# yuki-inaho/APDe-MVS

Measured on AMD Instinct MI355X. Metric: Mpix/s per PatchMatch iteration (ref view, N src) at 1/2/4/8 GPU; depth L1 vs ref, higher is better.
Workload: dtype f32

## Files before the change

### apde-mvs_amd/csrc/apd_kernels.hip

```cpp
#include <hip/hip_runtime.h>

#include <algorithm>
#include <cmath>
#include <cstdio>
#include <cstring>
#include <string>
#include <atomic>
#include <vector>

#include "../../include/apd_hip.h"
#include "apd_device.h"
#include <rocprim/device/device_scan.hpp>

using namespace apd;

#define WAVE 64
#define BLOCK 256
#define APD_PROF_SLOTS 64
#define APD_INSTR 32
#define APD_PROF_SPREAD 64
#define PROF_AT(ev, k) ((ev) + (k) + APD_PROF_SLOTS * (blockIdx.x & (APD_PROF_SPREAD - 1)))
#ifdef APD_PHASE_STAMPS
#define PHASE_STAMP(i)                                                                       \
    do {                                                                                     \
// ... 1876 lines not shown
        if (!live) continue;
        if (nwa) ++*nwa;
        if (inv == 0.0f) continue;
        const float c = ncc_finalize_pre(inv, srp, var, ss, sss, srs);
#pragma unroll
        for (int t = 0; t < 9; ++t) if (t == ns) sc[t] = c;
        ns++;
        strong_weight += 1.0f;
    }
    if (dead) return APD_COST_MAX;
    if (strong_weight <= 1e-6f) return center_cost;
    float mx = -1e10f;
#pragma unroll
    for (int t = 0; t < 9; ++t) if (t < ns && sc[t] > mx) mx = sc[t];
    float e[9];
    float sum = 0.0f;
#pragma unroll
    for (int t = 0; t < 9; ++t) {
        if (t < ns) { e[t] = d_expf(sc[t] - mx); sum += e[t]; }
    }
    float acc = 0.0f;
#pragma unroll
    for (int t = 0; t < 9; ++t) {
        if (t < ns) { float w = e[t] / sum; acc = fmaf(w, sc[t], acc); }
    }
    acc = (acc > APD_COST_MAX) ? APD_COST_MAX : acc;
    return (float)(0.25 * (double)center_cost + 0.75 * (double)acc);
}

#ifndef WV_WAVES
#define WV_WAVES 4
#endif
#ifndef WV_CUR_MATCH
#define WV_CUR_MATCH 1
#endif
#ifndef WV_P2_GEOM_BATCH
#define WV_P2_GEOM_BATCH 0
#endif
#define WV_BLOCK (WV_WAVES * WAVE)
__device__ __forceinline__ size_t cand_at(bool gm, int N, int v, int h, int wc, int wi, int li) {
    return gm ? ((size_t)(li / VM_P) * (size_t)(N * 8) + (size_t)(v * 8 + h)) * VM_P + (size_t)(li % VM_P)
              : ((size_t)v * 8 + h) * (size_t)wc + (size_t)wi;
}
#define GP_NO_FOCAL (-1.0f)
__device__ __forceinline__ float gp_focal(const float (&sc)[8]) {
    uint32_t pm = 0;
    float strong_weight = 0.0f;
#pragma unroll
    for (int k = 0; k < 8; ++k)
        if (sc[k] >= 0.0f) { pm |= 1u << k; strong_weight += 1.0f; }
    if (strong_weight <= 1e-6f) return GP_NO_FOCAL;
    float mx = -1e10f;
#pragma unroll
    for (int k = 0; k < 8; ++k) if (((pm >> k) & 1u) && sc[k] > mx) mx = sc[k];
    float e[8];
    float sum = 0.0f;
#pragma unroll
    for (int k = 0; k < 8; ++k) {
        e[k] = 0.0f;
        if ((pm >> k) & 1u) { e[k] = d_expf(sc[k] - mx); sum += e[k]; }
    }
    float acc = 0.0f;
#pragma unroll
    for (int k = 0; k < 8; ++k)
        if ((pm >> k) & 1u) { const float w = e[k] / sum; acc = fmaf(w, sc[k], acc); }
    acc = (acc > APD_COST_MAX) ? APD_COST_MAX : acc;
    return acc;
}
__device__ __forceinline__ float gp_final(bool dead, float centre_cost, float acc) {
    if (dead) return APD_COST_MAX;
    if (acc < 0.0f) return centre_cost;
    return (float)(0.25 * (double)centre_cost + 0.75 * (double)acc);
}
template <bool F16, bool SA> struct WvOcc {
#ifdef WV_LDS_OCC
    static constexpr int occ = WV_LDS_OCC;
#else
    static constexpr int occ = F16 ? 4 : 3;
#endif
    static constexpr bool pipe = occ < 4 && WV_CENTRE_PIPE;
};
template <bool F16, bool SA>
__global__ __launch_bounds__(WV_BLOCK, (WvOcc<F16, SA>::occ)) void k_sweep_weak_vm(Args a, const int *__restrict__ list, int count,
                                                                int iter, float *cand, int wc, int gm, int centre_in_sweep) {
    const int N = a.N, W = a.W;
    constexpr bool PIPE = WvOcc<F16, SA>::pipe;
    PHASE_BEGIN;
    const bool direct = cand != nullptr;
    WvLdsT<F16, 9, SA> &L = *reinterpret_cast<WvLdsT<F16, 9, SA> *>(apd_dyn_lds);
    wv_init_lut(L);
    float *costL = reinterpret_cast<float *>(&L + 1);
    uint8_t *wts = reinterpret_cast<uint8_t *>(costL + wv_cost_rows(N, direct) * VM_P);
    uint8_t *asl = wts + N * VM_P;
    const int VB = min(WV_P5_CHUNKS, N);
    const int blk = xcd_remap(blockIdx.x, gridDim.x);
    const int first = blk * VM_P;
    const int np = min(VM_P, count - first);
    const int tid = threadIdx.x;
    const int wave = __builtin_amdgcn_readfirstlane(tid >> 6), lane = tid & (WAVE - 1);
    const APD_C Cam &cam0 = a.cams[0];
    const bool geom = a.geom != 0;
    const float gf = a.gf;
    const int p1 = lane;
    const bool pv1 = p1 < np;
    const int c1 = list[first + min(p1, np - 1)];
    const int py1 = c1 / W, px1 = c1 - py1 * W;

    if (pv1) {
        const APD_G short2 *anc = a.anchors + (size_t)a.amap[c1] * 9;
        const int cid = a.sa_any ? a.sa[c1] : 0;
        const bool use_sa = cid != 0;
        if (wave == 0) {
            uint32_t hflag = 0, awin = 0;
            short2 ap[9];
#pragma unroll
            for (int k = 0; k < 9; ++k) ap[k] = anc[k];
            int lab[9], qk[9];
            uint8_t st[9];
            uint32_t sl[9];
#pragma unroll
            for (int k = 0; k < 9; ++k) {
                const bool ok = !(ap[k].x == -1 || ap[k].y == -1);
                qk[k] = ok ? ap[k].x + ap[k].y * W : c1;
                lab[k] = a.sa_any ? (int)a.sa[qk[k]] : cid;
                st[k] = a.weak[qk[k]];
                sl[k] = a.sel[qk[k]];
            }
            for (int v = 0; v < N; ++v) {
                uint32_t b = 0;
#pragma unroll
                for (int k = 1; k < 9; ++k) b |= ((sl[k] >> v) & 1u) << (k - 1);
                asl[v * VM_P + p1] = (uint8_t)b;
            }
            float4 hp[9];
#pragma unroll
            for (int k = 1; k < 9; ++k) hp[k] = a.plane[st[k] == APD_STRONG ? qk[k] : c1];
            const float4 cur = a.plane[c1];
#pragma unroll
            for (int k = 0; k < 9; ++k) {
                const bool ok = !(ap[k].x == -1 || ap[k].y == -1);
                L.anc[k * VM_P + p1] = ok ? ((int)(uint16_t)ap[k].x | ((int)ap[k].y << 16)) : -1;
                if (ok && !(use_sa && lab[k] != cid)) awin |= 1u << k;
                if (k >= 1 && ok && st[k] == APD_STRONG) {
                    hflag |= 1u << (k - 1);
                    L.hyp[(k - 1) * VM_P + p1] = hp[k];
                }
            }
            uint32_t cmatch = 0;
#pragma unroll
            for (int k = 8; k >= 1; --k)
                if (WV_CUR_MATCH && ((hflag >> (k - 1)) & 1u) && __float_as_uint(hp[k].x) == __float_as_uint(cur.x) &&
                    __float_as_uint(hp[k].y) == __float_as_uint(cur.y) && __float_as_uint(hp[k].z) == __float_as_uint(cur.z) &&
                    __float_as_uint(hp[k].w) == __float_as_uint(cur.w))
                    cmatch = (1u << 15) | ((uint32_t)(k - 1) << 12);
            L.flags[p1] = hflag | cmatch | (awin << 16) | (use_sa ? (1u << 29) : 0u);
            LANE_STAT(0, true);
            LANE_STAT(2, cmatch != 0);
#ifdef APD_PHASE_STAMPS
            {
                const float4 ft = a.fit[c1];
                auto same = [](float4 u, float4 w) {
                    return __float_as_uint(u.x) == __float_as_uint(w.x) && __float_as_uint(u.y) == __float_as_uint(w.y) &&
                           __float_as_uint(u.z) == __float_as_uint(w.z) && __float_as_uint(u.w) == __float_as_uint(w.w);
                };
                bool fc = false;
#pragma unroll
                for (int k = 1; k < 9; ++k) fc = fc || (((hflag >> (k - 1)) & 1u) && same(hp[k], ft));
                const bool has_fit = !(ft.x == 0 && ft.y == 0 && ft.z == 0);
                LANE_STAT(4, has_fit && same(ft, cur));
                LANE_STAT(6, has_fit && fc);
            }
#endif
            L.hyp[8 * VM_P + p1] = cur;
            L.pxy[p1] = px1 | (py1 << 16);
            int bx0 = px1, by0 = py1, bx1 = px1, by1 = py1;
#pragma unroll
            for (int k = 0; k < 9; ++k) {
                if (ap[k].x == -1 || ap[k].y == -1) continue;
                bx0 = min(bx0, (int)ap[k].x); bx1 = max(bx1, (int)ap[k].x);
                by0 = min(by0, (int)ap[k].y); by1 = max(by1, (int)ap[k].y);
            }
            L.box[p1] = (uint32_t)bx0 | ((uint32_t)by0 << 16);
            L.box[VM_P + p1] = (uint32_t)bx1 | ((uint32_t)by1 << 16);
        }
        wv_build_windows<F16>(a, L, p1, anc, cid, wave, WV_WAVES);
    }
    __syncthreads();
    PHASE_STAMP(0);

// ... 144 lines not shown
        if (G.valid) {
            wts[v * VM_P + p] = (uint8_t)w;
            if (G.v == 0) {
                const float4 fit = a.fit[c];
                L.st[2 * VM_P + p] = fcm;
                L.st[3 * VM_P + p] = wn;
                L.tsel[p] = tsel;
                uint32_t fl = (L.flags[p] & ~(7u << 25)) | ((uint32_t)mi << 25);
                if (!(fit.x == 0 && fit.y == 0 && fit.z == 0)) fl |= 1u << 31;
                L.flags[p] = fl;
                L.rng_n[p] = (uint16_t)rg.n;
            }
        }
    }
    __syncthreads();

    PHASE_STAMP(22);
    const int cur_row = direct ? 0 : 8 * N;
    const bool cur_shared = WV_CUR_MATCH && pv1 && ((L.flags[p1] >> 15) & 1u);
    for (int v = wave; v < N; v += WV_WAVES) {
        float val = 0.0f;
        const bool want = pv1 && wts[v * VM_P + p1] > 0 && !cur_shared;
        LANE_STAT(24, want);
        if (__ballot(want)) {
            const float4 pl = L.hyp[8 * VM_P + p1];
            const float kept = (iter == 0 && a.wcur && want) ? a.wcur[(size_t)v * a.HW + c1] : __int_as_float(0x7fc00000);
            const bool eval = want && __builtin_isnan(kept);
            float nv = kept;
            if (__ballot(eval)) {
                const float e = ncc_new_vm<F16, SA, true, 9, PIPE>(a, L, p1, px1, py1, v + 1, pl, eval, nullptr, &nwc, &nwa);
                if (eval) nv = e;
            }
            if (want) {
                val = nv;
                if (geom) val = fmaf(gf, geom_cost(a, px1, py1, v + 1, pl), val);
            }
        }
        if (!cur_shared) costL[(cur_row + v) * VM_P + p1] = val;
    }
    __syncthreads();

    if (wave == 0 && pv1) {
        const float wn = L.st[3 * VM_P + p1];
        float cost_now = 0.0f;
        for (int k = 0; k < N; ++k) {
            const int wk = wts[k * VM_P + p1];
            if (wk > 0) cost_now = fmaf((float)wk, costL[(cur_row + k) * VM_P + p1], cost_now);
        }
        cost_now /= wn;
        const float cost_init = cost_now;
        const int mi = (int)((L.flags[p1] >> 25) & 7u);
        const float fcm = L.st[2 * VM_P + p1];
        const float4 cur = L.hyp[8 * VM_P + p1];
        float depth_now = depth_from_plane(cam0, cur, px1, py1);
        float4 pnow = cur;
        bool taken = false;
        if ((L.flags[p1] >> mi) & 1u) {
            const float4 cnd = L.hyp[mi * VM_P + p1];
            const float db = depth_from_plane(cam0, cnd, px1, py1);
            if (db >= a.dmin && db <= a.dmax && fcm < cost_now) {
                depth_now = db; pnow = cnd; cost_now = fcm;
                a.sel[c1] = L.tsel[p1];
                taken = true;
            }
        }
        LANE_STAT(16, taken);
        L.pnow[p1] = pnow;
        L.st[0 * VM_P + p1] = depth_now;
        L.st[1 * VM_P + p1] = cost_now;
        L.st[2 * VM_P + p1] = cost_init;
    }
    __syncthreads();
    PHASE_STAMP(2);
    const bool refine = pv1 && (L.flags[p1] >> 31) != 0u;
    const float4 fit1 = a.fit[c1];
    uint32_t issued_nn = 0, issued_g = 0;

    float *part = reinterpret_cast<float *>(&L.hyp[5 * VM_P]);
    uint8_t *nxt = reinterpret_cast<uint8_t *>(part + 6 * VM_P);
    uint8_t *dead = nxt + 6 * VM_P;
    static_assert(6 * VM_P * (sizeof(float) + 2) <= 3 * VM_P * sizeof(float4), "early-exit state overlays hyp[5..7]");
    for (int i = tid; i < 6 * VM_P; i += WV_BLOCK) { part[i] = 0.0f; nxt[i] = 0; dead[i] = 0; }
    __syncthreads();
    auto fold = [&](int s, int K, int k, int row, int done) {
        for (int p = tid; p < VM_P; p += WV_BLOCK) {
            const int it = s * VM_P + p;
            if (dead[it]) continue;
            int v = nxt[it];
            float P = part[it];
            const int v0 = v;
            for (; v < N && v * K + k < done; ++v) {
                const int wk = wts[v * VM_P + p];
                if (wk > 0) P = fmaf((float)wk, costL[(row + v) * VM_P + p], P);
            }
            if (v == v0) continue;
            nxt[it] = (uint8_t)v;
            part[it] = P;
            if (P / L.st[3 * VM_P + p] >= L.st[1 * VM_P + p]) dead[it] = 1;
        }
    };

    for (int v0 = 0; v0 < N; v0 += WV_WAVES) {
        if (v0 > 0) fold(0, 1, 0, 0, v0);
        const int v = v0 + wave;
        if (v < N) {
            float cv = 0.0f;
            const bool want = refine && wts[v * VM_P + p1] > 0 && !dead[p1];
            LANE_STAT(22, want);
            const float4 fit = fit1;
            const float nv = ncc_new_vm<F16, SA, true, 9, PIPE>(a, L, p1, px1, py1, v + 1, fit, want, nullptr, &nwc, &nwa);
            if (want) {
                cv = nv;
                if (geom) cv = fmaf(gf, geom_cost(a, px1, py1, v + 1, fit), cv);
                ++issued_nn;
                issued_g += geom;
            }
            costL[v * VM_P + p1] = cv;
        }
        __syncthreads();
    }
    PHASE_STAMP(3);

    if (wave == 0 && refine) {
        const float wn = L.st[3 * VM_P + p1];
        float depth_now = L.st[0 * VM_P + p1], cost_now = L.st[1 * VM_P + p1];
        float4 pnow = L.pnow[p1];
        const float4 fit = fit1;
        if (!dead[p1]) {
            float tc = 0.0f;
            for (int kk = 0; kk < N; ++kk) {
                const int wk = wts[kk * VM_P + p1];
                if (wk > 0) tc = fmaf((float)wk, costL[kk * VM_P + p1], tc);
            }
            tc /= wn;
            const float db = depth_from_plane(cam0, fit, px1, py1);
            if (db >= a.dmin && db <= a.dmax && tc < cost_now) { depth_now = db; pnow = fit; cost_now = tc; }
        }
        Rng rg(a.seed_lo, a.seed_hi, (uint32_t)c1, ord_weak(iter));
        rg.n = L.rng_n[p1];
        if (rg.n & 3u) rg.refill();
        const Cands C = refine_candidates(a, px1, py1, rg, pnow, depth_now);
        for (int k = 0; k < 5; ++k) {
            float dk;
            float4 t = candidate(C, k, pnow, depth_now, dk);
            t.w = dist2origin(cam0, px1, py1, dk, t);
            WV_CAND(L)[k * VM_P + p1] = t;
        }
        L.pnow[p1] = pnow;
        L.st[0 * VM_P + p1] = depth_now;
        L.st[1 * VM_P + p1] = cost_now;
    }
    __syncthreads();
    PHASE_STAMP(4);

    {
        auto view_masks = [&](int v, uint64_t (&m)[5]) {
            const bool base = refine && wts[v * VM_P + p1] > 0;
#pragma unroll
            for (int k = 0; k < 5; ++k) m[k] = __ballot(base && !dead[(1 + k) * VM_P + p1]);
        };
        for (int v0 = 0; v0 < N;) {
            int v1 = v0, nch = 0, nne = 0;
            uint64_t ne = 0;
            while (v1 < N && nne < VB && nch < WV_P5_CHUNKS) {
                uint64_t m[5];
                view_masks(v1, m);
                int t = 0;
#pragma unroll
                for (int k = 0; k < 5; ++k) t += __builtin_popcountll(m[k]);
                nch += (t + WAVE - 1) / WAVE;
                if (t > 0) { ne |= 1ull << (v1 - v0); ++nne; }
                ++v1;
            }
            int g = 0;
            for (int v = v0; v < v1; ++v) {
                uint64_t m[5];
                view_masks(v, m);
                int off[6];
                off[0] = 0;
#pragma unroll
                for (int k = 0; k < 5; ++k) off[k + 1] = off[k] + __builtin_popcountll(m[k]);
                const int nv_items = off[5];
                for (int j = 0; j * WAVE < nv_items; ++j, ++g) {
                    if (g % WV_WAVES != wave) continue;
                    const int it = j * WAVE + lane;
                    const bool want = it < nv_items;
                    int k = 0;
#pragma unroll
                    for (int q = 1; q < 5; ++q) k += it >= off[q];
                    uint64_t mk = m[0];
#pragma unroll
                    for (int q = 1; q < 5; ++q) if (k == q) mk = m[q];
                    int pk = 0;
#pragma unroll
                    for (int q = 1; q < 5; ++q) if (k == q) pk = off[q];
                    const int p = want ? nth_set_bit(mk, it - pk) : p1;
                    const int pxy = L.pxy[p];
                    const int px = pxy & 0xFFFF, py = pxy >> 16;
                    const float4 tp = WV_CAND(L)[k * VM_P + p];
                    LANE_STAT(20, want);
                    const float nv = ncc_new_vm<F16, SA, true, 9, PIPE>(a, L, p, px, py, v + 1, tp, want, nullptr, &nwc, &nwa);
                    if (want) {
                        float cv = nv;
                        if (geom) cv = fmaf(gf, geom_cost(a, px, py, v + 1, tp), cv);
                        ++issued_nn;
                        issued_g += geom;
                        costL[(k * VB + __builtin_popcountll(ne & ((1ull << (v - v0)) - 1ull))) * VM_P + p] = cv;
                    }
                }
            }
            __syncthreads();
            for (int i = tid; i < 5 * VM_P; i += WV_BLOCK) {
                const int k = i / VM_P, p = i - k * VM_P, sl = (1 + k) * VM_P + p;
                if (dead[sl] || !(p < np && (L.flags[p] >> 31))) continue;
                int v = nxt[sl];
                float P = part[sl];
                for (; v < v1; ++v) {
                    const int wk = wts[v * VM_P + p];
                    if (wk > 0) P = fmaf((float)wk, costL[(k * VB + __builtin_popcountll(ne & ((1ull << (v - v0)) - 1ull))) * VM_P + p], P);
                }
                nxt[sl] = (uint8_t)v;
                part[sl] = P;
                if (P / L.st[3 * VM_P + p] >= L.st[1 * VM_P + p]) dead[sl] = 1;
            }
            __syncthreads();
            v0 = v1;
        }
    }
    PHASE_STAMP(5);

    if (a.evals && wave == 0) {
        uint32_t nn = 0, ng = 0;
        if (pv1) {
            int nsel = 0;
            for (int v = 0; v < N; ++v) nsel += wts[v * VM_P + p1] > 0;
            const int nh = __builtin_popcount(L.flags[p1] & 0xFFu);
            nn = (uint32_t)(nh * N + nsel);
            ng = geom ? (uint32_t)(nh * nsel + nsel) : 0u;
        }
#pragma unroll
        for (int o = 32; o > 0; o >>= 1) { nn += __shfl_xor(nn, o); ng += __shfl_xor(ng, o); }
        if (lane == 0) { atomicAdd(PROF_AT(a.evals, 1), (unsigned long long)nn); atomicAdd(PROF_AT(a.evals, 2), (unsigned long long)ng); }
    }
    if (a.evals) {
        uint32_t nn = issued_nn, ng = issued_g, wc0 = nwc, wa0 = nwa, wp0 = nwp;
#pragma unroll
        for (int o = 32; o > 0; o >>= 1) {
            nn += __shfl_xor(nn, o); ng += __shfl_xor(ng, o);
            wc0 += __shfl_xor(wc0, o); wa0 += __shfl_xor(wa0, o); wp0 += __shfl_xor(wp0, o);
        }
        if (lane == 0) {
            atomicAdd(PROF_AT(a.evals, 1), (unsigned long long)nn); atomicAdd(PROF_AT(a.evals, 2), (unsigned long long)ng);
            atomicAdd(PROF_AT(a.evals, 7), (unsigned long long)wc0); atomicAdd(PROF_AT(a.evals, 8), (unsigned long long)wa0);
            if (wp0) atomicAdd(PROF_AT(a.evals, 6), (unsigned long long)wp0);
        }
    }

    if (pv1) {
        for (int v = wave; v < N; v += WV_WAVES) a.vw[(size_t)v * a.HW + c1] = (uint8_t)wts[v * VM_P + p1];
        if (wave == 0) {
            float cost_now = L.st[1 * VM_P + p1];
            const float cost_init = L.st[2 * VM_P + p1], wn = L.st[3 * VM_P + p1];
            float4 pnow = L.pnow[p1];
            if (refine) {
                for (int k = 0; k < 5; ++k) {
                    if (dead[(1 + k) * VM_P + p1]) continue;
                    const float4 t = WV_CAND(L)[k * VM_P + p1];
                    const float tc = part[(1 + k) * VM_P + p1] / wn;
                    const float db = depth_from_plane(cam0, t, px1, py1);
                    if (db >= a.dmin && db <= a.dmax && tc < cost_now) { pnow = t; cost_now = tc; }
                }
            }
            if (a.state == APD_REFINE_INIT) {
                if ((double)cost_now < (double)cost_init - 0.1) { a.cost[c1] = cost_now; a.plane[c1] = pnow; }
                else a.cost[c1] = cost_init;
            } else {
                a.cost[c1] = cost_now;
                a.plane[c1] = pnow;
            }
        }
    }
    PHASE_STAMP(6);
}

#define PK_WAVES 8
#define PK_BLOCK (PK_WAVES * WAVE)
#ifndef PK_MINW
#define PK_MINW 1
#endif
#ifndef PK_PIPE
#define PK_PIPE true
#endif

#ifndef GP_CHUNK
#define GP_CHUNK 256
#endif
#ifndef GP_HS
#define GP_HS 8192
#endif
#define GP_CLOSE (GP_HS * 3 / 4 - 8 * GP_CHUNK)
static_assert(GP_CLOSE > 0 && GP_HS >= 256 && 256 % GP_CHUNK == 0, "k_gp_dedup table sizing");
#define GP_SMALL_N 64
#define GP_SMALL_HS 1024
#define GP_MEDIUM_HS 4096
static_assert(GP_SMALL_HS * 3 / 4 - 8 * GP_SMALL_N > 0 && 8 * GP_SMALL_N <= GP_SMALL_HS / 2, "small k_gp_dedup sizing");
#define GP_NONE 0xFFFFFFFFu

// ... 1282 lines not shown
        float Q[3];
        world_point(sc, sx, sy, src_depth, Q);
        float bx, by, refd;
        project_cam(Q, rc, bx, by, refd);
        const float dx = (float)px - bx, dy = (float)py - by;
        if (sqrtf(dx * dx + dy * dy) <= 2.0f) nc += 2;
        if (fabsf(rd - refd) / rd <= 0.02f) nc += 2;
    }
    if (nc > 255) nc = 255;
    a.conf[c] = (uint8_t)nc;
}

__global__ __launch_bounds__(BLOCK) void k_resize_nearest(const uint8_t *__restrict__ src, int sw, int sh,
                                                        uint8_t *__restrict__ dst, int dw, int dh, int elem) {
    const double ifx = 1.0 / ((double)dw / sw), ify = 1.0 / ((double)dh / sh);
    const size_t n = (size_t)dw * dh;
    for (size_t i = blockIdx.x * (size_t)BLOCK + threadIdx.x; i < n; i += (size_t)gridDim.x * BLOCK) {
        const int y = (int)(i / dw), x = (int)(i - (size_t)y * dw);
        const int sx = min((int)floor(x * ifx), sw - 1), sy = min((int)floor(y * ify), sh - 1);
        const uint8_t *s = src + ((size_t)sy * sw + sx) * elem;
        uint8_t *d = dst + i * elem;
        if (elem == 4) {
            *reinterpret_cast<uint32_t *>(d) = *reinterpret_cast<const uint32_t *>(s);
        } else if (elem == 16) {
            *reinterpret_cast<uint4 *>(d) = *reinterpret_cast<const uint4 *>(s);
        } else {
            for (int b = 0; b < elem; ++b) d[b] = s[b];
        }
    }
}

__global__ __launch_bounds__(BLOCK) void k_result_epilogue(const float4 *__restrict__ planes, size_t n, float dmin,
                                                         float dmax, float *__restrict__ depth_out,
                                                         float4 *__restrict__ planes_out) {
    for (size_t i = blockIdx.x * (size_t)BLOCK + threadIdx.x; i < n; i += (size_t)gridDim.x * BLOCK) {
        float4 p = planes[i];
        if (p.w < dmin || p.w > dmax) p.w = 0.0f;
        if (depth_out) depth_out[i] = p.w;
        if (planes_out) planes_out[i] = p;
    }
}

namespace {

struct DevBuf {
    void *p = nullptr;
    size_t bytes = 0;
};

const char *g_global_err = "";
std::string g_global_err_store;

void set_global_err(const std::string &s) {
    g_global_err_store = s;
    g_global_err = g_global_err_store.c_str();
}

}

struct apd_ctx {
    int device = 0;
    hipStream_t stream = nullptr;
    hipStream_t side[2] = {nullptr, nullptr};
    hipEvent_t ev_fork = nullptr, ev_side[2] = {nullptr, nullptr};
    bool overlap = true;
    std::string err;
    DevBuf imgs, quad, depth, views, cams, plane, cost, sel, sel2, vw, weak, conf, sa, amap, anchors, reliable, nearest,
        fit, curve, lists, rowcnt, rowoff, totals, near_off, dargs, evals, near_ring, near_g, wcand, lrs, wcur, arec, ga_stage,
        wlist, gp_cb, gp_cnt, gp_cur, gp_refs, gp_ccnt, gp_cbase, gp_plist, gp_pidx, gp_pcost, gp_tmp, dpairs, gp_cls;
    int n_near = 0;
    int host_stat[4] = {0, 0, 0, 0};
    int near_levels = 0;
    Args args{};
    bool loaded = false, prepared = false;
    int optional_fallbacks = 0;
    bool prep_timed = false;
    int dw_tile_w = 8;
    int tile_w = 16;
    bool cand_pairs = true;
    bool weak_per_colour = false;
    bool weak_quad = false;
    bool cand_gm = true;
    bool centre_in_sweep = false;
    bool gp_on = false;
    bool ga_split = true;
    bool rec_on = false;
    bool dtex = true;
    int gp_np = 0;
    bool gp_one_pass = true;
    bool gp_async = true;
    bool gp_pending = false;
    size_t gp_pcap = 0;
    int ncu = 256;
    bool gp_place = true;
    bool gp_small = true;
    int gp_cap_factor = 2;
    bool lr_handover = true;
    bool wcur_on = true;
    bool wcur_fresh = false;
    int weak_count = 0;
    size_t lrs_need = 0;
    int cnt[4] = {0, 0, 0, 0};
    size_t list_cap = 0;
    bool want_curve = false;
    apd_params params{};
    hipEvent_t ev[16] = {};
    apd_timing timing{};
    struct ProfEv {
        hipEvent_t e0, e1;
        int kind;
        int64_t px;
    };
    bool prof = false;
    std::vector<ProfEv> prof_ev;
    std::vector<hipEvent_t> prof_pool;
};

#define HIP_OK(ctx, call)                                                                          \
    do {                                                                                           \
        hipError_t e_ = (call);                                                                    \
        if (e_ != hipSuccess) {                                                                    \
            (ctx)->err = std::string(#call) + ": " + hipGetErrorString(e_);                        \
            return APD_EDEVICE;                                                                    \
        }                                                                                          \
    } while (0)

static int ensure(apd_ctx *ctx, DevBuf &b, size_t bytes) {
    if (bytes == 0) bytes = 16;
    if (b.bytes >= bytes) return APD_OK;
    if (b.p) (void)hipFree(b.p);
    b.p = nullptr;
    b.bytes = 0;
    if (hipMalloc(&b.p, bytes) != hipSuccess) {
        ctx->err = "hipMalloc(" + std::to_string(bytes) + ") failed";
        return APD_ENOMEM;
    }
    b.bytes = bytes;
    return APD_OK;
}

static int check_launch(apd_ctx *ctx, const char *what) {
    hipError_t e = hipGetLastError();
    if (e != hipSuccess) {
        ctx->err = std::string("launch ") + what + ": " + hipGetErrorString(e);
        return APD_EDEVICE;
    }
    return APD_OK;
}

static void precompute_views(const apd_camera *cams, int ni, SrcView *views, Args &a) {
    const apd_camera &r = cams[0];
    const double kr0 = r.K[0], kr2 = r.K[2], kr4 = r.K[4], kr5 = r.K[5];
    const double Kri[9] = {1.0 / kr0, 0.0, -kr2 / kr0, 0.0, 1.0 / kr4, -kr5 / kr4, 0.0, 0.0, 1.0};
    a.ikx = (float)(1.0 / kr0);
    a.iky = (float)(1.0 / kr4);
    a.cxk = (float)(kr2 / kr0);
    a.cyk = (float)(kr5 / kr4);
    double rC[3];
    for (int j = 0; j < 3; ++j)
        rC[j] = -((double)r.R[j] * r.t[0] + (double)r.R[3 + j] * r.t[1] + (double)r.R[6 + j] * r.t[2]);
    for (int s = 0; s < ni; ++s) {
        const apd_camera &c = cams[s];
        double sC[3], Crel[3], trel[3], Rrel[9];
        for (int j = 0; j < 3; ++j)
            sC[j] = -((double)c.R[j] * c.t[0] + (double)c.R[3 + j] * c.t[1] + (double)c.R[6 + j] * c.t[2]);
        for (int i = 0; i < 3; ++i)
// ... 69 lines not shown
    };
    uint32_t lo = 0u, hi = 0x7f800000u;
    if (!reach(hi)) return false;
    while (lo < hi) {
        const uint32_t mid = lo + (hi - lo) / 2u;
        if (reach(mid)) hi = mid;
        else lo = mid + 1u;
    }
    std::memcpy(limit, &lo, 4);
    return true;
}

static void drain(apd_ctx *ctx) {
    (void)hipStreamSynchronize(ctx->stream);
    for (auto &ss : ctx->side)
        if (ss) (void)hipStreamSynchronize(ss);
}

static inline unsigned blocks_for(size_t n, int per_block) { return (unsigned)((n + per_block - 1) / per_block); }

extern "C" {

int32_t apd_abi_version(void) { return APD_ABI_VERSION; }

int32_t apd_device_count(void) {
    int n = 0;
    if (hipGetDeviceCount(&n) != hipSuccess) return 0;
    return n;
}

apd_ctx *apd_create(int32_t device) {
    int n = 0;
    if (hipGetDeviceCount(&n) != hipSuccess || n <= 0) {
        set_global_err("no HIP device visible");
        return nullptr;
    }
    if (device < 0 || device >= n) {
        set_global_err("device index out of range");
        return nullptr;
    }
    if (hipSetDevice(device) != hipSuccess) {
        set_global_err("hipSetDevice failed");
        return nullptr;
    }
    apd_ctx *ctx = new apd_ctx();
    ctx->device = device;
    if (hipStreamCreateWithFlags(&ctx->stream, hipStreamNonBlocking) != hipSuccess) {
        set_global_err("hipStreamCreate failed");
        delete ctx;
        return nullptr;
    }
    for (auto &e : ctx->ev) (void)hipEventCreateWithFlags(&e, hipEventDisableSystemFence);
    int prio_least = 0, prio_greatest = 0;
    (void)hipDeviceGetStreamPriorityRange(&prio_least, &prio_greatest);
    const bool low_side = !(getenv("APD_SIDE_PRIORITY") && atoi(getenv("APD_SIDE_PRIORITY")) == 0);
    if (low_side && prio_least <= 0 && prio_greatest < 0) {
        hipStream_t hi = nullptr;
        if (hipStreamCreateWithPriority(&hi, hipStreamNonBlocking, prio_greatest) == hipSuccess) {
            (void)hipStreamDestroy(ctx->stream);
            ctx->stream = hi;
        }
    }
    if (getenv("APD_DEBUG_PRIO")) fprintf(stderr, "apd: stream priorities least %d greatest %d\n", prio_least, prio_greatest);
    for (auto &ss : ctx->side) {
        int prio = 0;
        if (low_side && prio_least > 0 && &ss == &ctx->side[0]) prio = prio_least;
        if (low_side && prio_least <= 0 && prio_greatest < 0 && &ss == &ctx->side[1]) prio = prio_greatest;
        if (hipStreamCreateWithPriority(&ss, hipStreamNonBlocking, prio) != hipSuccess) {
            set_global_err("hipStreamCreate failed");
            for (auto &t : ctx->side) if (t) (void)hipStreamDestroy(t);
            (void)hipStreamDestroy(ctx->stream);
            delete ctx;
            return nullptr;
        }
    }
    (void)hipEventCreateWithFlags(&ctx->ev_fork, hipEventDisableTiming);
    for (auto &e : ctx->ev_side) (void)hipEventCreateWithFlags(&e, hipEventDisableTiming);
    ctx->overlap = getenv("APD_NO_OVERLAP") == nullptr;
    ctx->cand_pairs = getenv("APD_NO_CAND_PAIRS") == nullptr;
    ctx->weak_per_colour = getenv("APD_WEAK_PER_COLOUR") != nullptr;
    ctx->weak_quad = getenv("APD_WEAK_QUAD") != nullptr;
    ctx->cand_gm = getenv("APD_NO_CAND_GROUP_MAJOR") == nullptr && !ctx->weak_per_colour;
    ctx->centre_in_sweep = getenv("APD_CAND_CENTRE_IN_SWEEP") != nullptr;
    ctx->ga_split = getenv("APD_NO_GA_SPLIT") == nullptr;
    ctx->lr_handover = getenv("APD_NO_LR_HANDOVER") == nullptr;
    ctx->wcur_on = getenv("APD_NO_WCUR") == nullptr;
    ctx->dtex = getenv("APD_NO_DTEX") == nullptr;
    ctx->gp_one_pass = getenv("APD_GP_TWO_PASS") == nullptr;
    ctx->gp_small = getenv("APD_GP_NO_SMALL") == nullptr;
    ctx->gp_place = getenv("APD_GP_FILL") == nullptr;
    ctx->gp_async = getenv("APD_GP_SYNC") == nullptr && ctx->gp_one_pass && ctx->gp_small && ctx->gp_place;
    {
        int n = 0;
        if (hipDeviceGetAttribute(&n, hipDeviceAttributeMultiprocessorCount, device) == hipSuccess && n > 0) ctx->ncu = n;
    }
    if (const char *e = getenv("APD_GP_CAP_FACTOR")) ctx->gp_cap_factor = std::max(0, std::min(8, atoi(e)));

    if (const char *e = getenv("APD_DW_TILE_W")) {
        const int t = atoi(e);
        if (t == 1 || t == 2 || t == 4 || t == 8 || t == 16 || t == 32 || t == 64) ctx->dw_tile_w = t;
    }
    if (const char *e = getenv("APD_TILE_W")) {
        const int t = atoi(e);
        if (t == 4 || t == 8 || t == 16 || t == 32 || t == 64) ctx->tile_w = t;
    }
    const void *vm_kernels[] = {
        (const void *)k_sweep_strong_vm<true, false>, (const void *)k_sweep_strong_vm<false, false>,
        (const void *)k_sweep_strong_vm<true, true>, (const void *)k_sweep_strong_vm<false, true>,
        (const void *)k_sweep_weak_vm<true, false>, (const void *)k_sweep_weak_vm<false, false>,
        (const void *)k_sweep_weak_vm<true, true>, (const void *)k_sweep_weak_vm<false, true>,
        (const void *)k_depth_to_weak_vm<true, false>, (const void *)k_depth_to_weak_vm<false, false>,
        (const void *)k_depth_to_weak_vm<true, true>, (const void *)k_depth_to_weak_vm<false, true>,
        (const void *)k_depth_to_weak_vm<true, false, true>, (const void *)k_depth_to_weak_vm<true, true, true>,
        (const void *)k_local_refine_vm<true, false>, (const void *)k_local_refine_vm<false, false>,
        (const void *)k_local_refine_vm<true, true>, (const void *)k_local_refine_vm<false, true>,
        (const void *)k_random_init_vm<true, false, false>, (const void *)k_random_init_vm<false, false, false>,
        (const void *)k_random_init_vm<true, true, false>, (const void *)k_random_init_vm<false, true, false>,
        (const void *)k_random_init_vm<true, false, true>, (const void *)k_random_init_vm<false, false, true>,
        (const void *)k_random_init_vm<true, true, true>, (const void *)k_random_init_vm<false, true, true>};
    for (const void *k : vm_kernels) (void)hipFuncSetAttribute(k, hipFuncAttributeMaxDynamicSharedMemorySize, 160 * 1024);
    return ctx;
}

void apd_destroy(apd_ctx *ctx) {
    if (!ctx) return;
    (void)hipSetDevice(ctx->device);
    drain(ctx);
    DevBuf *bufs[] = {&ctx->imgs, &ctx->quad, &ctx->depth, &ctx->views, &ctx->cams, &ctx->plane, &ctx->cost,
                      &ctx->sel, &ctx->sel2, &ctx->vw, &ctx->weak, &ctx->conf, &ctx->sa, &ctx->amap, &ctx->anchors,
                      &ctx->reliable, &ctx->nearest, &ctx->fit, &ctx->curve, &ctx->lists, &ctx->rowcnt,
                      &ctx->rowoff, &ctx->totals, &ctx->near_off, &ctx->dargs, &ctx->evals, &ctx->near_ring, &ctx->near_g, &ctx->wcand, &ctx->arec, &ctx->ga_stage,
                      &ctx->lrs, &ctx->wcur, &ctx->wlist, &ctx->gp_cb, &ctx->gp_cnt, &ctx->gp_cur, &ctx->gp_refs, &ctx->gp_ccnt,
                      &ctx->gp_cbase, &ctx->gp_plist, &ctx->gp_pidx, &ctx->gp_pcost, &ctx->gp_tmp, &ctx->dpairs, &ctx->gp_cls};
    for (DevBuf *b : bufs)
        if (b->p) (void)hipFree(b->p);
    for (auto &e : ctx->ev) (void)hipEventDestroy(e);
    for (auto &pe : ctx->prof_ev) { (void)hipEventDestroy(pe.e0); (void)hipEventDestroy(pe.e1); }
    for (hipEvent_t e : ctx->prof_pool) (void)hipEventDestroy(e);
    for (auto &ss : ctx->side) if (ss) { (void)hipStreamSynchronize(ss); (void)hipStreamDestroy(ss); }
    if (ctx->ev_fork) (void)hipEventDestroy(ctx->ev_fork);
    for (auto &e : ctx->ev_side) if (e) (void)hipEventDestroy(e);
    (void)hipStreamDestroy(ctx->stream);
    delete ctx;
}

const char *apd_last_error(const apd_ctx *ctx) { return ctx ? ctx->err.c_str() : g_global_err; }

static bool try_ensure(apd_ctx *ctx, DevBuf &b, size_t bytes) {
    if (ensure(ctx, b, bytes) == APD_OK) return true;
    (void)hipGetLastError();
    ctx->err.clear();
    if (ctx->optional_fallbacks++ < 8)
        fprintf(stderr, "apd: optional device buffer of %zu bytes not allocated on device %d: its exact fallback path runs\n",
                bytes, ctx->device);
    return false;
}

int32_t apd_set_problem(apd_ctx *ctx, const apd_problem *pb) {
    if (!ctx || !pb) return APD_EINVAL;
    (void)hipSetDevice(ctx->device);
    drain(ctx);
    ctx->loaded = ctx->prepared = ctx->prep_timed = false;
    const int W = pb->width, H = pb->height, NI = pb->num_images;
    if (NI > APD_MAX_IMAGES) { ctx->err = "num_images > 32"; return APD_ETOOMANYVIEWS; }
    if (W < 1 || H < 1 || NI < 2 || !pb->images || !pb->cameras) { ctx->err = "bad problem dimensions"; return APD_EINVAL; }
    if (W > 32767 || H > 32767 || (size_t)W * H > (size_t)1 << 30) { ctx->err = "image too large"; return APD_EINVAL; }
// ... 580 lines not shown
    int st;
    APD_G unsigned long long *evals = (ctx->prof && ctx->evals.p) ? (APD_G unsigned long long *)ctx->evals.p : nullptr;
    for (int colour = 0; colour < 2; ++colour) {
        const int n = ctx->cnt[colour];
        if (n <= 0) continue;
        hipEvent_t e0 = prof_begin(ctx);
        Args ak = a;
        ak.evals = evals;
        if (!(ctx->wcur_fresh && iter == 0)) ak.wcur = nullptr;
        LAUNCH_TEX_SA(k_sweep_strong_vm, dim3(blocks_for((size_t)n, VM_P)), dim3(VM_BLOCK), vm_lds_bytes(a.N, ctx->args.tex_f16 != 0) + sa_lds_bytes(a), s,
                      ak, (const int *)list_ptr(ctx, colour), n, iter);
        prof_end(ctx, e0, APD_PROF_STRONG_SWEEP, n);
        if ((st = check_launch(ctx, "k_sweep_strong"))) return st;
    }
    if (a.use_apd) {
        hipEvent_t ewp = prof_begin(ctx);
        const bool centre_kernel = !ctx->centre_in_sweep;
        hipStream_t sr = s, sg = s;
        if (ctx->overlap) {
            HIP_OK(ctx, hipEventRecord(ctx->ev_fork, s));
            HIP_OK(ctx, hipStreamWaitEvent(ctx->side[0], ctx->ev_fork, 0));
            sr = ctx->side[0];
            if (centre_kernel) {
                HIP_OK(ctx, hipStreamWaitEvent(ctx->side[1], ctx->ev_fork, 0));
                sg = ctx->side[1];
            }
        }
        hipEvent_t e0 = prof_begin(ctx, sr);
        hipLaunchKernelGGL(k_ransac_fit, dim3(blocks_for((size_t)a.HW, BLOCK)), dim3(BLOCK), 0, sr, a, iter);
        prof_end(ctx, e0, APD_PROF_RANSAC_FIT, a.HW, sr);
        if (ctx->overlap) HIP_OK(ctx, hipEventRecord(ctx->ev_side[0], sr));
        const int nw = ctx->cnt[2] + ctx->cnt[3];
        const int wc = std::max(ctx->weak_count, 1);
        float *cand = nullptr;
        const int gm = ctx->cand_gm ? 1 : 0;
        if (ctx->cand_pairs && nw > 0 && ctx->gp_on) {
            if (ctx->wcand.bytes < wcand_bytes(a.N, (size_t)wc, nw) || ctx->wlist.bytes < (size_t)nw * sizeof(int)) {
                ctx->err = "candidate cost buffers not sized by apd_stage_prepare";
                return APD_ESTATE;
            }
            Args ac = a;
            ac.evals = evals;
            {
                hipEvent_t e1 = prof_begin(ctx, sg);
                if (ctx->gp_np > 0)
                    LAUNCH_TEX_SA(k_gp_cost, dim3(blocks_for((size_t)ctx->gp_np, BLOCK)), dim3(BLOCK), gp_cost_lds_bytes(a.N), sg, ac,
                               (const int2 *)ctx->gp_plist.p, ctx->gp_np, (float *)ctx->gp_pcost.p);
                prof_end(ctx, e1, APD_PROF_GP_COST, ctx->gp_np, sg);
                if (centre_kernel) {
                    if (ctx->overlap) HIP_OK(ctx, hipEventRecord(ctx->ev_side[1], sg));
                    e1 = prof_begin(ctx);
                    LAUNCH_TEX_SA(k_weak_cand_g, dim3(blocks_for((size_t)nw, VM_P)), dim3(PK_BLOCK), 0, s, ac, (const int *)ctx->wlist.p, nw,
                                  (const uint8_t *)ctx->gp_cb.p, (float *)ctx->wcand.p, wc, gm);
                    prof_end(ctx, e1, APD_PROF_WEAK_CAND_G, nw);
                    if (ctx->overlap) HIP_OK(ctx, hipStreamWaitEvent(s, ctx->ev_side[1], 0));
                }
                e1 = prof_begin(ctx);
                hipLaunchKernelGGL(k_weak_cand_comb, dim3(2 * blocks_for((size_t)nw, VM_P)), dim3(BLOCK), 0, s, ac,
                                   (const int *)ctx->wlist.p, nw, (const uint8_t *)ctx->gp_cb.p, (const uint8_t *)ctx->gp_cb.p + wc,
                                   (const uint32_t *)ctx->gp_pidx.p, (const float *)ctx->gp_pcost.p, (float *)ctx->wcand.p, wc, gm,
                                   centre_kernel ? 0 : 1);
                prof_end(ctx, e1, APD_PROF_WEAK_CAND_COMB, nw);
            }
            cand = (float *)ctx->wcand.p;
        }
        if (ctx->overlap) HIP_OK(ctx, hipStreamWaitEvent(s, ctx->ev_side[0], 0));
        if (!ctx->weak_per_colour && nw > 0 && ctx->wlist.bytes < (size_t)nw * sizeof(int)) {
            ctx->err = "WEAK lists not built by apd_stage_prepare";
            return APD_ESTATE;
        }
        for (int colour = 0; colour < (ctx->weak_per_colour ? 2 : 1); ++colour) {
            const int n = ctx->weak_per_colour ? ctx->cnt[2 + colour] : nw;
            const int *wl = ctx->weak_per_colour ? (const int *)list_ptr(ctx, 2 + colour) : (const int *)ctx->wlist.p;
            if (n <= 0) continue;
            Args aw = a;
            aw.evals = evals;
            if (!(ctx->wcur_fresh && iter == 0)) aw.wcur = nullptr;
            e0 = prof_begin(ctx);
            const bool direct = cand != nullptr;
            LAUNCH_TEX_SA(k_sweep_weak_vm, dim3(blocks_for((size_t)n, VM_P)), dim3(WV_BLOCK),
                          (ctx->args.tex_f16 ? (ctx->args.sa_any ? wv_lds_bytes<true, 9, true>(a.N, direct) : wv_lds_bytes<true, 9, false>(a.N, direct))
                                             : (ctx->args.sa_any ? wv_lds_bytes<false, 9, true>(a.N, direct) : wv_lds_bytes<false, 9, false>(a.N, direct))),
                          s,
                          aw, wl, n, iter, cand, wc, gm, (direct && !centre_kernel) ? 1 : 0);
            prof_end(ctx, e0, APD_PROF_WEAK_SWEEP, n);
        }
        prof_end(ctx, ewp, APD_PROF_WEAK_PATH, ctx->cnt[2] + ctx->cnt[3]);
        if ((st = check_launch(ctx, "weak sweep"))) return st;
    }
    ctx->wcur_fresh = false;
    return APD_OK;
}

int32_t apd_stage_finish(apd_ctx *ctx) {
    if (!ctx || !ctx->prepared) return APD_ESTATE;
    (void)hipSetDevice(ctx->device);
    Args a = ctx->args;
    hipStream_t s = ctx->stream;
    int st;
    const unsigned gpx = blocks_for((size_t)a.HW, BLOCK);
    hipLaunchKernelGGL(k_depth_normal, dim3(gpx), dim3(BLOCK), 0, s, a);
    for (int colour = 0; colour < 2; ++colour) {
        const int n = ctx->cnt[colour];
        if (n > 0)
            hipLaunchKernelGGL(k_filter, dim3(blocks_for((size_t)n, BLOCK)), dim3(BLOCK), 0, s, a,
                               (const int *)list_ptr(ctx, colour), n);
    }
    if (ctx->want_curve && ctx->curve.p) a.curve = devptr<decltype(a.curve)>(ctx->curve.p);
    a.lr_ncc = nullptr;
    a.lr_geo = nullptr;
    if (ctx->lr_handover && ctx->lrs_need > 0 && ctx->lrs.p && ctx->lrs.bytes >= ctx->lrs_need) {
        const size_t plane = ctx->lrs_need / (sizeof(float) * (a.geom ? 2 : 1));
        a.lr_ncc = devptr<decltype(a.lr_ncc)>(ctx->lrs.p);
        a.lr_geo = a.geom ? devptr<decltype(a.lr_geo)>((float *)ctx->lrs.p + plane) : nullptr;
    }
    {
        const int tw = ctx->dw_tile_w, th = VM_P / tw;
        const unsigned nb = (unsigned)(((a.W + tw - 1) / tw) * ((a.H + th - 1) / th));
        const int dwc = dw_chunk(a.N, a.geom != 0, sa_lds_bytes(a));
        Args ad = a;
        ad.evals = (ctx->prof && ctx->evals.p) ? (APD_G unsigned long long *)ctx->evals.p : nullptr;
        const bool dp = a.dpairs != nullptr;
        hipEvent_t e0 = prof_begin(ctx);
        if (dp) {
            const size_t lds = dw_lds_bytes(a.N, a.geom != 0, dwc) + sa_lds_bytes(a);
            if (a.sa_any) hipLaunchKernelGGL((k_depth_to_weak_vm<true, true, true>), dim3(nb), dim3(VM_BLOCK), lds, s, ad, dwc, tw);
            else hipLaunchKernelGGL((k_depth_to_weak_vm<true, false, true>), dim3(nb), dim3(VM_BLOCK), lds, s, ad, dwc, tw);
        } else {
            LAUNCH_TEX_SA(k_depth_to_weak_vm, dim3(nb), dim3(VM_BLOCK), dw_lds_bytes(a.N, a.geom != 0, dwc) + sa_lds_bytes(a), s, ad, dwc, tw);
        }
        prof_end(ctx, e0, APD_PROF_DEPTH_TO_WEAK, a.HW);
    }
    if (a.geom || a.use_apd) hipLaunchKernelGGL(k_confidence, dim3(gpx), dim3(BLOCK), 0, s, a);
    {
        const int tw = ctx->dw_tile_w, th = VM_P / tw;
        const unsigned nb = (unsigned)(((a.W + tw - 1) / tw) * ((a.H + th - 1) / th));
        LAUNCH_TEX_SA(k_local_refine_vm, dim3(nb), dim3(VM_BLOCK), lr_lds_bytes(a.N) + sa_lds_bytes(a), s, a, lr_chunk(a.N), tw);
    }
    if ((st = check_launch(ctx, "finish"))) return st;
    return APD_OK;
}

static void prepare_timing(apd_ctx *ctx, apd_timing &t) {
    memset(&t, 0, sizeof(t));
    if (!ctx->prep_timed) return;
    (void)hipEventElapsedTime(&t.anchors_ms, ctx->ev[0], ctx->ev[1]);
    (void)hipEventElapsedTime(&t.lists_ms, ctx->ev[1], ctx->ev[14]);
    (void)hipEventElapsedTime(&t.pairs_ms, ctx->ev[14], ctx->ev[2]);
    (void)hipEventElapsedTime(&t.join_ms, ctx->ev[2], ctx->ev[3]);
    (void)hipEventElapsedTime(&t.prepare_ms, ctx->ev[0], ctx->ev[3]);
    (void)hipEventElapsedTime(&t.init_ms, ctx->ev[1], ctx->ev[15]);
}

int32_t apd_get_prepare_timing(apd_ctx *ctx, apd_timing *timing) {
    if (!ctx || !timing) return APD_EINVAL;
    if (!ctx->prepared) return APD_ESTATE;
    (void)hipSetDevice(ctx->device);
    HIP_OK(ctx, hipStreamSynchronize(ctx->stream));
    prepare_timing(ctx, *timing);
    return APD_OK;
}

int32_t apd_run_patchmatch(apd_ctx *ctx) {
    if (!ctx || !ctx->loaded) return APD_ESTATE;
    (void)hipSetDevice(ctx->device);
    int st;
    hipStream_t s = ctx->stream;
// ... 261 lines not shown
```

Measured before the change: 69.04.

## Precompute geometric costs so early-exit bound includes remaining geom tail

In the weak-pixel sweep, the geometric consistency cost for every view and hypothesis is computed up front and stored in the candidate buffer. The early-exit fold then adds the weighted remaining geometric terms to the partial cost, giving a tighter lower bound so hypotheses are killed before their expensive NCC evaluations. The NCC loop reads the stored geometric value instead of recomputing it. In exchange, geometric costs are now computed even for views that would have been skipped, and extra barriers and global buffer traffic are added.

```diff
diff --git a/apde-mvs_amd/csrc/apd_kernels.hip b/apde-mvs_amd/csrc/apd_kernels.hip
--- a/apde-mvs_amd/csrc/apd_kernels.hip
+++ b/apde-mvs_amd/csrc/apd_kernels.hip
@@ -1982,7 +1982,8 @@
 };
 template <bool F16, bool SA>
 __global__ __launch_bounds__(WV_BLOCK, (WvOcc<F16, SA>::occ)) void k_sweep_weak_vm(Args a, const int *__restrict__ list, int count,
-                                                                int iter, float *cand, int wc, int gm, int centre_in_sweep) {
+                                                                int iter, float *cand, int wc, int gm, int centre_in_sweep,
+                                                                int geom_tail_on) {
     const int N = a.N, W = a.W;
     constexpr bool PIPE = WvOcc<F16, SA>::pipe;
     PHASE_BEGIN;
@@ -2005,6 +2006,10 @@
     const bool pv1 = p1 < np;
     const int c1 = list[first + min(p1, np - 1)];
     const int py1 = c1 / W, px1 = c1 - py1 * W;
+    const bool gtail = geom && direct && geom_tail_on != 0;
+    auto gt_at = [&](int v, int s, int p) -> float * {
+        return cand + cand_at(gm != 0, N, v, s, wc, gm ? 0 : a.amap[list[first + p]], first + p);
+    };
 
     if (pv1) {
         const APD_G short2 *anc = a.anchors + (size_t)a.amap[c1] * 9;
@@ -2315,7 +2320,15 @@
     static_assert(6 * VM_P * (sizeof(float) + 2) <= 3 * VM_P * sizeof(float4), "early-exit state overlays hyp[5..7]");
     for (int i = tid; i < 6 * VM_P; i += WV_BLOCK) { part[i] = 0.0f; nxt[i] = 0; dead[i] = 0; }
     __syncthreads();
-    auto fold = [&](int s, int K, int k, int row, int done) {
+    auto tail = [&](int s, int p, int v, float P) {
+        float T = P;
+        for (; v < N; ++v) {
+            const int wk = wts[v * VM_P + p];
+            if (wk > 0) T = fmaf((float)wk, fmaf(gf, *gt_at(v, s, p), 0.0f), T);
+        }
+        return T;
+    };
+    auto fold = [&](int s, int K, int k, int row, int done, bool all) {
         for (int p = tid; p < VM_P; p += WV_BLOCK) {
             const int it = s * VM_P + p;
             if (dead[it]) continue;
@@ -2326,15 +2339,31 @@
                 const int wk = wts[v * VM_P + p];
                 if (wk > 0) P = fmaf((float)wk, costL[(row + v) * VM_P + p], P);
             }
-            if (v == v0) continue;
+            if (v == v0 && !all) continue;
             nxt[it] = (uint8_t)v;
             part[it] = P;
-            if (P / L.st[3 * VM_P + p] >= L.st[1 * VM_P + p]) dead[it] = 1;
+            float T = P;
+            if (gtail && p < np && (L.flags[p] >> 31)) T = tail(s, p, v, P);
+            if (T / L.st[3 * VM_P + p] >= L.st[1 * VM_P + p]) dead[it] = 1;
         }
     };
 
+    if (gtail) {
+        for (int v = wave; v < N; v += WV_WAVES) {
+            if (refine && wts[v * VM_P + p1] > 0) {
+                *gt_at(v, 0, p1) = geom_cost(a, px1, py1, v + 1, fit1);
+                ++issued_g;
+            }
+        }
+        __syncthreads();
+        fold(0, 1, 0, 0, 0, true);
+        __syncthreads();
+        PHASE_STAMP(10);
+    }
+
     for (int v0 = 0; v0 < N; v0 += WV_WAVES) {
-        if (v0 > 0) fold(0, 1, 0, 0, v0);
+        if (v0 > 0) fold(0, 1, 0, 0, v0, false);
+        if (v0 > 0 && gtail) __syncthreads();
         const int v = v0 + wave;
         if (v < N) {
             float cv = 0.0f;
@@ -2344,9 +2373,9 @@
             const float nv = ncc_new_vm<F16, SA, true, 9, PIPE>(a, L, p1, px1, py1, v + 1, fit, want, nullptr, &nwc, &nwa);
             if (want) {
                 cv = nv;
-                if (geom) cv = fmaf(gf, geom_cost(a, px1, py1, v + 1, fit), cv);
+                if (gtail) cv = fmaf(gf, *gt_at(v, 0, p1), cv);
+                else if (geom) { cv = fmaf(gf, geom_cost(a, px1, py1, v + 1, fit), cv); ++issued_g; }
                 ++issued_nn;
-                issued_g += geom;
             }
             costL[v * VM_P + p1] = cv;
         }
@@ -2392,57 +2421,7 @@
 #pragma unroll
             for (int k = 0; k < 5; ++k) m[k] = __ballot(base && !dead[(1 + k) * VM_P + p1]);
         };
-        for (int v0 = 0; v0 < N;) {
-            int v1 = v0, nch = 0, nne = 0;
-            uint64_t ne = 0;
-            while (v1 < N && nne < VB && nch < WV_P5_CHUNKS) {
-                uint64_t m[5];
-                view_masks(v1, m);
-                int t = 0;
-#pragma unroll
-                for (int k = 0; k < 5; ++k) t += __builtin_popcountll(m[k]);
-                nch += (t + WAVE - 1) / WAVE;
-                if (t > 0) { ne |= 1ull << (v1 - v0); ++nne; }
-                ++v1;
-            }
-            int g = 0;
-            for (int v = v0; v < v1; ++v) {
-                uint64_t m[5];
-                view_masks(v, m);
-                int off[6];
-                off[0] = 0;
-#pragma unroll
-                for (int k = 0; k < 5; ++k) off[k + 1] = off[k] + __builtin_popcountll(m[k]);
-                const int nv_items = off[5];
-                for (int j = 0; j * WAVE < nv_items; ++j, ++g) {
-                    if (g % WV_WAVES != wave) continue;
-                    const int it = j * WAVE + lane;
-                    const bool want = it < nv_items;
-                    int k = 0;
-#pragma unroll
-                    for (int q = 1; q < 5; ++q) k += it >= off[q];
-                    uint64_t mk = m[0];
-#pragma unroll
-                    for (int q = 1; q < 5; ++q) if (k == q) mk = m[q];
-                    int pk = 0;
-#pragma unroll
-                    for (int q = 1; q < 5; ++q) if (k == q) pk = off[q];
-                    const int p = want ? nth_set_bit(mk, it - pk) : p1;
-                    const int pxy = L.pxy[p];
-                    const int px = pxy & 0xFFFF, py = pxy >> 16;
-                    const float4 tp = WV_CAND(L)[k * VM_P + p];
-                    LANE_STAT(20, want);
-                    const float nv = ncc_new_vm<F16, SA, true, 9, PIPE>(a, L, p, px, py, v + 1, tp, want, nullptr, &nwc, &nwa);
-                    if (want) {
-                        float cv = nv;
-                        if (geom) cv = fmaf(gf, geom_cost(a, px, py, v + 1, tp), cv);
-                        ++issued_nn;
-                        issued_g += geom;
-                        costL[(k * VB + __builtin_popcountll(ne & ((1ull << (v - v0)) - 1ull))) * VM_P + p] = cv;
-                    }
-                }
-            }
-            __syncthreads();
+        auto fold5 = [&](int v0, int v1, uint64_t ne) {
             for (int i = tid; i < 5 * VM_P; i += WV_BLOCK) {
                 const int k = i / VM_P, p = i - k * VM_P, sl = (1 + k) * VM_P + p;
                 if (dead[sl] || !(p < np && (L.flags[p] >> 31))) continue;
@@ -2454,8 +2433,86 @@
                 }
                 nxt[sl] = (uint8_t)v;
                 part[sl] = P;
-                if (P / L.st[3 * VM_P + p] >= L.st[1 * VM_P + p]) dead[sl] = 1;
-            }
+                const float T = gtail ? tail(1 + k, p, v, P) : P;
+                if (T / L.st[3 * VM_P + p] >= L.st[1 * VM_P + p]) dead[sl] = 1;
+            }
+        };
+        if (gtail) {
+            float Pw[5][3];
+            if (refine) {
+#pragma unroll
+                for (int k = 0; k < 5; ++k) geom_point(a, px1, py1, WV_CAND(L)[k * VM_P + p1], Pw[k]);
+            }
+            for (int v = wave; v < N; v += WV_WAVES) {
+                if (refine && wts[v * VM_P + p1] > 0) {
+                    GeomHead gh[5];
+                    float sdep[5];
+#pragma unroll
+                    for (int k = 0; k < 5; ++k) gh[k] = geom_head(a, v + 1, Pw[k]);
+#pragma unroll
+                    for (int k = 0; k < 5; ++k) sdep[k] = a.depth[gh[k].idx];
+#pragma unroll
+                    for (int k = 0; k < 5; ++k) *gt_at(v, 1 + k, p1) = geom_tail(a, px1, py1, v + 1, gh[k], sdep[k]);
+                    issued_g += 5;
+                }
+            }
+            __syncthreads();
+            fold5(0, 0, 0);
+            __syncthreads();
+            PHASE_STAMP(11);
+        }
+        for (int v0 = 0; v0 < N;) {
+            int v1 = v0, nch = 0, nne = 0;
+            uint64_t ne = 0;
+            while (v1 < N && nne < VB && nch < WV_P5_CHUNKS) {
+                uint64_t m[5];
+                view_masks(v1, m);
+                int t = 0;
+#pragma unroll
+                for (int k = 0; k < 5; ++k) t += __builtin_popcountll(m[k]);
+                nch += (t + WAVE - 1) / WAVE;
+                if (t > 0) { ne |= 1ull << (v1 - v0); ++nne; }
+                ++v1;
+            }
+            int g = 0;
+            for (int v = v0; v < v1; ++v) {
+                uint64_t m[5];
+                view_masks(v, m);
+                int off[6];
+                off[0] = 0;
+#pragma unroll
+                for (int k = 0; k < 5; ++k) off[k + 1] = off[k] + __builtin_popcountll(m[k]);
+                const int nv_items = off[5];
+                for (int j = 0; j * WAVE < nv_items; ++j, ++g) {
+                    if (g % WV_WAVES != wave) continue;
+                    const int it = j * WAVE + lane;
+                    const bool want = it < nv_items;
+                    int k = 0;
+#pragma unroll
+                    for (int q = 1; q < 5; ++q) k += it >= off[q];
+                    uint64_t mk = m[0];
+#pragma unroll
+                    for (int q = 1; q < 5; ++q) if (k == q) mk = m[q];
+                    int pk = 0;
+#pragma unroll
+                    for (int q = 1; q < 5; ++q) if (k == q) pk = off[q];
+                    const int p = want ? nth_set_bit(mk, it - pk) : p1;
+                    const int pxy = L.pxy[p];
+                    const int px = pxy & 0xFFFF, py = pxy >> 16;
+                    const float4 tp = WV_CAND(L)[k * VM_P + p];
+                    LANE_STAT(20, want);
+                    const float nv = ncc_new_vm<F16, SA, true, 9, PIPE>(a, L, p, px, py, v + 1, tp, want, nullptr, &nwc, &nwa);
+                    if (want) {
+                        float cv = nv;
+                        if (gtail) cv = fmaf(gf, *gt_at(v, 1 + k, p), cv);
+                        else if (geom) { cv = fmaf(gf, geom_cost(a, px, py, v + 1, tp), cv); ++issued_g; }
+                        ++issued_nn;
+                        costL[(k * VB + __builtin_popcountll(ne & ((1ull << (v - v0)) - 1ull))) * VM_P + p] = cv;
+                    }
+                }
+            }
+            __syncthreads();
+            fold5(v0, v1, ne);
             __syncthreads();
             v0 = v1;
         }
@@ -3904,6 +3961,7 @@
     bool weak_quad = false;
     bool cand_gm = true;
     bool centre_in_sweep = false;
+    bool geom_tail = true;
     bool gp_on = false;
     bool ga_split = true;
     bool rec_on = false;
@@ -4139,6 +4197,7 @@
     ctx->weak_quad = getenv("APD_WEAK_QUAD") != nullptr;
     ctx->cand_gm = getenv("APD_NO_CAND_GROUP_MAJOR") == nullptr && !ctx->weak_per_colour;
     ctx->centre_in_sweep = getenv("APD_CAND_CENTRE_IN_SWEEP") != nullptr;
+    ctx->geom_tail = getenv("APD_NO_GEOM_TAIL") == nullptr;
     ctx->ga_split = getenv("APD_NO_GA_SPLIT") == nullptr;
     ctx->lr_handover = getenv("APD_NO_LR_HANDOVER") == nullptr;
     ctx->wcur_on = getenv("APD_NO_WCUR") == nullptr;
@@ -4885,7 +4944,7 @@
                           (ctx->args.tex_f16 ? (ctx->args.sa_any ? wv_lds_bytes<true, 9, true>(a.N, direct) : wv_lds_bytes<true, 9, false>(a.N, direct))
                                              : (ctx->args.sa_any ? wv_lds_bytes<false, 9, true>(a.N, direct) : wv_lds_bytes<false, 9, false>(a.N, direct))),
                           s,
-                          aw, wl, n, iter, cand, wc, gm, (direct && !centre_kernel) ? 1 : 0);
+                          aw, wl, n, iter, cand, wc, gm, (direct && !centre_kernel) ? 1 : 0, ctx->geom_tail ? 1 : 0);
             prof_end(ctx, e0, APD_PROF_WEAK_SWEEP, n);
         }
         prof_end(ctx, ewp, APD_PROF_WEAK_PATH, ctx->cnt[2] + ctx->cnt[3]);
```

After: 75.48 (median of 6 runs). 1.09x the previous value.
